# rsadsb/dump1090_rs

Hardware: AMD Instinct MI355X
Metric: IQ Msamples/s demodulated (higher is better)
Workload: dtype i16 IQ -> f32 magnitude (exact) -> u16/i32 integer

## Files before the change

dump1090_rs_amd/csrc/adsb_aux.hip:

```cpp
#include <algorithm>

#include "../../include/adsb_hip.h"
#include "adsb_dev_common.h"
#include "adsb_scan_geometry.h"
#include "adsb_tail_dev.h"
#include "adsb_fix_dev.h"

namespace adsb {

namespace {


__global__ __launch_bounds__(256) void k_to_mag(const uint32_t *__restrict__ iq, uint32_t n,
                                                uint16_t *__restrict__ data)
{
    const uint32_t t = blockIdx.x * 256u + threadIdx.x;
    const uint32_t i0 = 8u * t;
    if (i0 >= (uint32_t)kMagDataLen) return;
    const __amdgpu_buffer_rsrc_t rsrc = __builtin_amdgcn_make_buffer_rsrc((void *)iq, 0, (int)(n * 4u), 0x00020000);
    uint32_t w[8];
#pragma unroll
    for (int i = 0; i < 8; i++) {
        int off = ((int)i0 + i - kLead) * 4;
        asm volatile("" : "+v"(off));
        w[i] = __builtin_amdgcn_raw_buffer_load_b32(rsrc, off, 0, 0);
    }
    uint32_t pk[4];
#pragma unroll
    for (int i = 0; i < 4; i++) pk[i] = mag2(w[2 * i], w[2 * i + 1]);
    if (i0 + 8u <= (uint32_t)kMagDataLen) {
        *(uint4 *)(data + i0) = make_uint4(pk[0], pk[1], pk[2], pk[3]);
    } else {
        for (uint32_t i = 0; i0 + i < (uint32_t)kMagDataLen; i++) data[i0 + i] = (uint16_t)(pk[i >> 1] >> (16 * (i & 1)));
    }
}

__global__ __launch_bounds__(256) void k_to_mag_u8(const uint8_t *__restrict__ iq, uint32_t n, const uint16_t *__restrict__ tab,
                                                   uint16_t *__restrict__ data)
{
    const uint32_t t = blockIdx.x * 256u + threadIdx.x;
    const uint32_t i0 = 8u * t;
    if (i0 >= (uint32_t)kMagDataLen) return;
    const __amdgpu_buffer_rsrc_t rsrc = __builtin_amdgcn_make_buffer_rsrc((void *)iq, 0, (int)(n * 2u), 0x00020000);
    uint32_t w[8];
#pragma unroll
    for (int i = 0; i < 8; i++) w[i] = load_u8_sample(rsrc, (int)i0 + i - kLead, (int)n, tab);
    uint32_t pk[4];
#pragma unroll
    for (int i = 0; i < 4; i++) pk[i] = mag2(w[2 * i], w[2 * i + 1]);
    if (i0 + 8u <= (uint32_t)kMagDataLen) {
        *(uint4 *)(data + i0) = make_uint4(pk[0], pk[1], pk[2], pk[3]);
    } else {
        for (uint32_t i = 0; i0 + i < (uint32_t)kMagDataLen; i++) data[i0 + i] = (uint16_t)(pk[i >> 1] >> (16 * (i & 1)));
    }
}

__global__ __launch_bounds__(256) void k_widen_u8(const uint8_t *__restrict__ src, unsigned long long first, uint32_t count,
                                                  const uint16_t *__restrict__ tab, uint32_t *__restrict__ dst)
{
    const uint32_t i = blockIdx.x * 256u + threadIdx.x;
    if (i >= count) return;
    const uint8_t *b = src + 2ull * (first + i);
    dst[i] = widen_u8_pair(tab, (uint32_t)b[0] | (uint32_t)b[1] << 8);
}

__global__ __launch_bounds__(256) void k_reset(Counters *ctr, uint32_t *bitmap, uint32_t lg)
{
    const uint32_t i = blockIdx.x * blockDim.x + threadIdx.x;
    constexpr uint32_t kCtrDwords = sizeof(Counters) / 4;
    if (i < kCtrDwords) ((uint32_t *)ctr)[i] = 0;
    if (bitmap) bitmap_clear(bitmap, lg, i, gridDim.x * blockDim.x);
}


__global__ __launch_bounds__(256) void k_match(ScanParams p)
{
    if (p.order_cnt) TAIL_PRIO();
    __shared__ uint32_t stab[3 * 256];
    __shared__ uint32_t coarse[kCoarseWords];
    for (int i = threadIdx.x; i < 3 * 256; i += blockDim.x) stab[i] = p.tables[kTabX56 * 256 + i];
    if (threadIdx.x < kCoarseWords) coarse[threadIdx.x] = p.bitmap[bitmap_words(p.bitmap_lg) + threadIdx.x];
    __syncthreads();
    const uint32_t seg_cap = p.seg_cap;
    const bool is_dap = blockIdx.x >= (uint32_t)kApWaveSegs / 2;
    uint32_t n[2];
    const uint64_t *ap[2];
    uint32_t first = 0, stride = 2 * blockDim.x;
    if (is_dap) {
        n[0] = n[1] = min(p.ctr->n_dap, p.dap_cap);
        ap[0] = ap[1] = p.dap;
        first = (blockIdx.x - kApWaveSegs / 2) * 4 * blockDim.x;
        stride = (gridDim.x - kApWaveSegs / 2) * 4 * blockDim.x;
    } else {
        for (int h = 0; h < 2; h++) {
            const uint32_t sg = 2 * blockIdx.x + h;
            n[h] = min(p.ctr->seg_ap[sg], seg_cap);
            ap[h] = p.ap + (uint64_t)sg * seg_cap;
        }
    }
    const uint32_t nmax = max(n[0], n[1]);
    for (uint32_t i0 = first + threadIdx.x; i0 < nmax; i0 += stride) {
        uint64_t e[4];
        uint32_t c[4];
#pragma unroll
        for (int k = 0; k < 4; k++) {
            const int h = is_dap ? 0 : k >> 1;
            const uint32_t i = i0 + (is_dap ? (uint32_t)k : (uint32_t)(k & 1)) * blockDim.x;
            e[k] = i < n[h] ? ap[h][i] : ~0ull;
        }
#pragma unroll
        for (int k = 0; k < 4; k++) {
            const uint32_t code = entry_code(e[k]);
            c[k] = entry_value(e[k]);
            if (code >= 5 && code < 10) c[k] = gf_apply(stab, c[k]);
        }
#pragma unroll
        for (int k = 0; k < 4; k++) {
            if (e[k] == ~0ull || !((coarse[(c[k] & 4095u) >> 5] >> (c[k] & 31)) & 1u)) continue;
            const uint32_t at = bitmap_index(c[k], p.bitmap_lg);
            if ((p.bitmap[at >> 5] >> (at & 31)) & 1u) {
                const uint32_t idx = atomicAdd(&p.ctr->n_hits, 1u);
                if (p.order_cnt) {
                    const uint32_t ch = (uint32_t)entry_chunk(e[k]), tl = entry_j(e[k]) / (uint32_t)fastgeo::kTile;
                    const uint32_t at = atomicAdd(&p.order_cnt[ch * fastgeo::kTilesPerChunk + tl], 1u);
                    if (at < kTileBucket) {
                        const size_t place = (size_t)ch * kOrderBucket + tl * kTileBucket + at;
                        p.order_tmp[place] = e[k];
                        if (p.hit_fields) p.hit_fields[place * kHitFieldWords + 5] = 0u;
                    } else {
                        atomicOr(&p.ctr->overflow, 1u);
                    }
                } else if (idx < p.hits_cap) {
                    p.hits[idx] = e[k];
                    if (p.hit_fields) p.hit_fields[(size_t)idx * kHitFieldWords + 5] = 0u;
                } else {
                    atomicOr(&p.ctr->overflow, 1u);
                }
            }
        }
    }
}


__global__ __launch_bounds__(1024) void k_order_prefix(ScanParams p)
{
    TAIL_PRIO();
    __shared__ uint32_t part[1024];
    __shared__ uint32_t carry;
    const uint32_t tid = threadIdx.x;
    constexpr uint32_t T = fastgeo::kTilesPerChunk;
    if (p.ctr->overflow) {
        for (uint32_t c = tid; c < p.n_chunks * T; c += 1024) p.order_cnt[c] = 0;
        return;
    }
    if (tid == 0) carry = 0;
    __syncthreads();
    for (uint32_t c0 = 0; c0 <= p.n_chunks; c0 += 1024) {
        const uint32_t c = c0 + tid;
        uint32_t v = 0;
        if (c < p.n_chunks)
#pragma unroll
            for (uint32_t t = 0; t < T; t++) v += min(p.order_cnt[c * T + t], kTileBucket);
        part[tid] = v;
        __syncthreads();
        for (uint32_t off = 1; off < 1024; off <<= 1) {
            const uint32_t add = tid >= off ? part[tid - off] : 0u;
            __syncthreads();
            part[tid] += add;
            __syncthreads();
        }
        if (c <= p.n_chunks) p.order_base[c] = carry + part[tid] - v;
        __syncthreads();
        if (tid == 1023) carry += part[1023];
        __syncthreads();
    }
}



__device__ __forceinline__ uint32_t score_hash_first(const ScoreDev &sd, uint32_t v)
{
    uint32_t h = score_hash_slot(v) & sd.hash_mask;
    for (;;) {
        const unsigned long long cur = __hip_atomic_load(&sd.hash[h], __ATOMIC_RELAXED, __HIP_MEMORY_SCOPE_AGENT);
        if (cur == ~0ull) return 0xFFFFFFFFu;
        if ((uint32_t)(cur >> 32) == v) return (uint32_t)cur;
        h = (h + 1u) & sd.hash_mask;
    }
}

__device__ __forceinline__ bool score_in_filter(const ScoreDev &sd, uint32_t v, uint32_t i)
{
    if (v == 0) return true;
    if ((sd.exact[v >> 5] >> (v & 31)) & 1u) return true;
    if (sd.earlier && ((sd.earlier[v >> 5] >> (v & 31)) & 1u)) return true;
    return score_hash_first(sd, v) < i;
}

__device__ __forceinline__ int score_repair(const ScoreDev &sd, uint32_t i, uint32_t damaged, const uint32_t *tables, uint32_t fix,
                                            uint32_t *repair)
{
    const TrialRecord &r = sd.rec[i];
    const uint32_t df = (uint32_t)r.msg[0] >> 3;
    if (df != 17u && df != 18u) return -2;
    const uint32_t ab = fix_lookup(tables, (uint32_t)(r.power >> 40), fix);
    if (ab == kFixNoRepair) return -2;
    *repair = ab;
    const uint32_t a = ab & 0xFFu, b = ab >> 8;
    const uint32_t addr = damaged ^ fix_addr_mask(a) ^ fix_addr_mask(b);
    if (!score_in_filter(sd, addr, i)) return -1;
    return a == kFixNoBit ? ADSB_SCORE_FIXED_1BIT : ADSB_SCORE_FIXED_2BIT;
}

__device__ __forceinline__ int score_trial(const ScoreDev &sd, uint32_t i, uint32_t *adds, const uint32_t *tables, uint32_t fix,
                                           uint32_t *repair)
{
    const uint32_t w = sd.si[i], v = w & 0xFFFFFFu, kind = w >> 24;
    *adds = 0;
    switch (kind) {
    case kSkApShort: return score_in_filter(sd, v, i) ? 1000 : -1;
    case kSkApLong: return score_in_filter(sd, v, i) ? 1000 : -2;
    case kSkDf11: return score_in_filter(sd, v, i) ? 1000 : -1;
    case kSkDf11Iid0:
        if (score_in_filter(sd, v, i)) return 1600;
        *adds = v;
        return 750;
    case kSkDf17:
        if (score_in_filter(sd, v, i)) return 1800;
        *adds = v;
        return 1400;
    case kSkDf18:
        if (score_in_filter(sd, v, i)) return 1800;
        *adds = v | (1u << 25);
        return 1400;
    case kSkNone: return -3;
    case kSkOther: return fix ? score_repair(sd, i, v, tables, fix, repair) : -2;
    default: return -2;
    }
}


__global__ __launch_bounds__(256) void k_score(ScanParams p)
{
    TAIL_PRIO();
    const ScoreDev &sd = p.score;
    const uint32_t n = sd.state->n;
    const uint32_t per = (n + gridDim.x - 1) / gridDim.x;
    const uint32_t first = blockIdx.x * per, last = min(n, first + per);
    uint32_t emits = 0, addc = 0;
    for (uint32_t i = first + threadIdx.x; i < last; i += blockDim.x) {
        const uint64_t pos = sd.pos[i];
        uint32_t g0 = i;
        while (g0 > 0 && i - g0 < 8 && sd.pos[g0 - 1] == pos) g0--;
        int best = -2, mine = -2;
        uint32_t win = 0xFFFFFFFFu, my_add = 0, my_fix = kFixNoRepair;
        for (uint32_t k = g0; k < n && k < g0 + 16 && sd.pos[k] == pos; k++) {
            uint32_t a, fx = kFixNoRepair;
            const int s = score_trial(sd, k, &a, p.tables, p.fix, &fx);
            if (k == i) {
                mine = s;
                my_add = a;
                my_fix = fx;
            }
            if (s > best) {
                best = s;
                win = k;
            }
        }
        const bool emit = win == i && best >= 0;
        const uint32_t fa = my_fix & 0x7Fu, fb = (my_fix >> 8) & 0x7Fu;
        sd.flag[i] = (emit ? 1u : 0u) | (my_add ? 2u : 0u) | ((uint32_t)(mine + 3) << 8) | (fa >> 6) << 2 | (fa & 63u) << 19 | fb << 25;
        emits += emit;
        addc += my_add != 0;
    }
    __shared__ uint32_t tot[2];
    if (threadIdx.x < 2) tot[threadIdx.x] = 0;
    __syncthreads();
    if (emits) atomicAdd(&tot[0], emits);
    if (addc) atomicAdd(&tot[1], addc);
    __syncthreads();
    if (threadIdx.x < 2) sd.blk[2 * blockIdx.x + threadIdx.x] = tot[threadIdx.x];
}

__global__ __launch_bounds__(256) void k_emit(ScanParams p)
{
    TAIL_PRIO();
    const ScoreDev &sd = p.score;
    const uint32_t n = sd.state->n;
    const uint32_t per = (n + gridDim.x - 1) / gridDim.x;
    const uint32_t first = blockIdx.x * per, last = min(n, first + per);
    static_assert(kScoreBlocks == 256, "the block-offset reduction below takes one earlier block per thread");
    __shared__ uint32_t base[2], scan[2][256];
    __shared__ unsigned long long stage[5 * 256];
    __shared__ uint32_t wtot[2][4];
    {
// ... 93 lines not shown
        if (threadIdx.x == 0) {
            base[0] += scan[0][255];
            base[1] += scan[1][255];
        }
        __syncthreads();
    }
    asm volatile("s_waitcnt vmcnt(0)" ::: "memory");
#pragma unroll
    for (int off = 32; off > 0; off >>= 1) my_sum += __shfl_down(my_sum, off);
    if ((threadIdx.x & 63) == 0 && my_sum) atomicAdd(&sd.state->msg_sum, my_sum);
    asm volatile("s_waitcnt vmcnt(0)" ::: "memory");
    __shared__ bool is_last;
    __syncthreads();
    if (threadIdx.x == 0) is_last = atomicAdd(&sd.state->blocks_done, 1u) == gridDim.x - 1;
    __syncthreads();
    if (!is_last) return;
    __shared__ uint32_t tot[2][4];
    {
        uint32_t nm = threadIdx.x < gridDim.x ? sd.blk[2 * threadIdx.x] : 0u;
        uint32_t na = threadIdx.x < gridDim.x ? sd.blk[2 * threadIdx.x + 1] : 0u;
#pragma unroll
        for (int off = 32; off > 0; off >>= 1) {
            nm += __shfl_down(nm, off);
            na += __shfl_down(na, off);
        }
        if ((threadIdx.x & 63) == 0) {
            tot[0][threadIdx.x >> 6] = nm;
            tot[1][threadIdx.x >> 6] = na;
        }
    }
    __syncthreads();
    if (threadIdx.x == 0) {
        const uint32_t nm = tot[0][0] + tot[0][1] + tot[0][2] + tot[0][3];
        const uint32_t na = tot[1][0] + tot[1][1] + tot[1][2] + tot[1][3];
        const unsigned long long ms = atomicAdd(&sd.state->msg_sum, 0ull);
        uint32_t *sm = (uint32_t *)sd.summary;
        const uint32_t vals[8] = {nm, na, (uint32_t)ms, (uint32_t)(ms >> 32), sd.state->scored, 0u, 0u, sd.seq};
#pragma unroll
        for (int k = 0; k < 8; k++) host_store32(sm + k, vals[k]);
        sd.state->n = 0;
        sd.state->scored = 0;
        sd.state->blocks_done = 0;
        sd.state->msg_sum = 0;
    }
}


template <bool FROM_MAG, bool BUCKETS, bool U8 = false>
__global__ __launch_bounds__(256) void k_records(ScanParams p, TrialRecord *rec)
{
    if (p.order_cnt) TAIL_PRIO();
    extern __shared__ uint64_t sorted[];
    records_block<FROM_MAG, BUCKETS, false, U8>(p, rec, blockIdx.x, gridDim.x, sorted, true);
}

__global__ __launch_bounds__(kCarrySamples) void k_update_carry(const uint32_t *__restrict__ prev,
                                                               const uint32_t *__restrict__ src, long long n,
                                                               uint32_t *__restrict__ next)
{
    const long long i = threadIdx.x, idx = n - kCarrySamples + i;
    next[i] = idx >= 0 ? src[idx] : prev[i + n];
}

__global__ __launch_bounds__(kCarrySamples) void k_update_carry_u8(const uint32_t *__restrict__ prev,
                                                                  const uint8_t *__restrict__ src, long long n,
                                                                  const uint16_t *__restrict__ tab, uint32_t *__restrict__ next)
{
    const long long i = threadIdx.x, idx = n - kCarrySamples + i;
    next[i] = idx >= 0 ? widen_u8_pair(tab, (uint32_t)src[2 * idx] | (uint32_t)src[2 * idx + 1] << 8) : prev[i + n];
}

__global__ __launch_bounds__(64) void k_shard_summary(ScanParams p)
{
    if (threadIdx.x != 0) return;
    uint32_t *sm = (uint32_t *)p.summary;
    const uint32_t vals[9] = {p.ctr->n_hits, p.ctr->overflow, p.ctr->fresh_sum, p.ctr->n_fresh, 0u, 0u, 0u, p.seq, 0u};
    host_store32(sm + 9, summary_check(vals));
    host_store32(sm + 8, 0u);
#pragma unroll
    for (int k = 0; k < 8; k++) host_store32(sm + k, vals[k]);
}

__global__ __launch_bounds__(256) void k_set_addresses(const uint32_t *__restrict__ addrs, uint32_t n,
                                                       uint32_t *bitmap, uint32_t lg)
{
    const uint32_t i = blockIdx.x * blockDim.x + threadIdx.x;
    if (i < n) bitmap_set(bitmap, lg, addrs[i] & 0xFFFFFFu);
}

__global__ __launch_bounds__(256) void k_mag_digest(uint32_t first_bits, uint32_t count,
                                                    unsigned long long *out)
{
    unsigned long long sum = 0, h = 0;
    const uint32_t half = (count + 1) / 2;
    for (uint32_t i = blockIdx.x * blockDim.x + threadIdx.x; i < half; i += gridDim.x * blockDim.x) {
        const uint32_t b0 = first_bits + i, b1 = first_bits + i + half;
        const f32x2 x = {__uint_as_float(b0), __uint_as_float(i + half < count ? b1 : 0u)};
        const uint32_t pk = mag_tail2(x);
        const uint32_t u0 = pk & 0xFFFFu, u1 = pk >> 16;
        sum += u0;
        h ^= ((unsigned long long)u0 + 1ull) * (2ull * b0 + 1ull);
        if (i + half < count) {
            sum += u1;
            h ^= ((unsigned long long)u1 + 1ull) * (2ull * b1 + 1ull);
        }
    }
    atomicAdd(&out[0], sum);
    atomicXor(&out[1], h);
}

__global__ __launch_bounds__(256) void k_fix_lookup(const uint32_t *__restrict__ tables, const uint32_t *__restrict__ residuals,
                                                    uint32_t n, uint32_t mode, uint32_t *__restrict__ out)
{
    const uint32_t i = blockIdx.x * blockDim.x + threadIdx.x;
    if (i < n) out[i] = fix_lookup(tables, residuals[i], mode);
}

inline int hip_ok(hipError_t e) { return e == hipSuccess ? 0 : (int)e; }
inline void hip_clear() { (void)hipGetLastError(); }

}

int launch_to_mag(const void *d_iq, uint32_t n, uint16_t *d_data, void *stream, const uint16_t *u8_table)
{
    hip_clear();
    const int blocks = ((kMagDataLen + 7) / 8 + 255) / 256;
    if (u8_table) {
        hipLaunchKernelGGL(k_to_mag_u8, dim3(blocks), dim3(256), 0, (hipStream_t)stream, (const uint8_t *)d_iq, n, u8_table, d_data);
        return hip_ok(hipGetLastError());
    }
    hipLaunchKernelGGL(k_to_mag, dim3(blocks), dim3(256), 0, (hipStream_t)stream,
                       (const uint32_t *)d_iq, n, d_data);
    return hip_ok(hipGetLastError());
}

int launch_widen_u8(const void *d_src, uint64_t first, uint32_t count, const uint16_t *u8_table, uint32_t *dst, void *stream)
{
    hip_clear();
    if (count == 0) return 0;
    hipLaunchKernelGGL(k_widen_u8, dim3((count + 255) / 256), dim3(256), 0, (hipStream_t)stream, (const uint8_t *)d_src,
                       (unsigned long long)first, count, u8_table, dst);
    return hip_ok(hipGetLastError());
}

int launch_reset(Counters *ctr, uint32_t *bitmap, uint32_t bitmap_lg, void *stream)
{
    hip_clear();
    const uint32_t ctr_blocks = (uint32_t)((sizeof(Counters) / 4 + 255) / 256);
    const uint32_t blocks = bitmap ? std::max(ctr_blocks, std::min(512u, bitmap_alloc_words(bitmap_lg) / 4 / 256 + 1u)) : ctr_blocks;
    hipLaunchKernelGGL(k_reset, dim3(blocks), dim3(256), 0, (hipStream_t)stream, ctr, bitmap, bitmap_lg);
    return hip_ok(hipGetLastError());
}

int launch_match(const ScanParams &p, void *stream)
{
    hip_clear();
    const uint32_t blocks = kApWaveSegs / 2 + 64;
    hipLaunchKernelGGL(k_match, dim3(blocks), dim3(256), 0, (hipStream_t)stream, p);
    return hip_ok(hipGetLastError());
}

int launch_records(const ScanParams &p, SrcFormat fmt, TrialRecord *d_rec, void *stream)
{
    hip_clear();
    uint32_t blocks = p.n_chunks + 8u;
    if (blocks > 1024) blocks = 1024;
    if (fmt == SrcFormat::kCu8) {
        if (!p.u8_table) return (int)hipErrorInvalidValue;
        if (p.order_cnt)
            hipLaunchKernelGGL((k_records<false, true, true>), dim3(blocks), dim3(256), kOrderBucket * (sizeof(uint64_t) + sizeof(uint16_t)),
                               (hipStream_t)stream, p, d_rec);
        else
            hipLaunchKernelGGL((k_records<false, false, true>), dim3(blocks), dim3(256), 0, (hipStream_t)stream, p, d_rec);
    } else if (fmt == SrcFormat::kMag)
        hipLaunchKernelGGL((k_records<true, false>), dim3(blocks), dim3(256), 0, (hipStream_t)stream, p, d_rec);
    else if (p.order_cnt)
        hipLaunchKernelGGL((k_records<false, true>), dim3(blocks), dim3(256), kOrderBucket * (sizeof(uint64_t) + sizeof(uint16_t)),
                           (hipStream_t)stream, p, d_rec);
    else
        hipLaunchKernelGGL((k_records<false, false>), dim3(blocks), dim3(256), 0, (hipStream_t)stream, p, d_rec);
    return hip_ok(hipGetLastError());
}

int launch_order_hits(const ScanParams &p, void *stream)
{
    hip_clear();
    if (!p.order_cnt || !p.order_base || !p.order_tmp) return 0;
    hipLaunchKernelGGL(k_order_prefix, dim3(1), dim3(1024), 0, (hipStream_t)stream, p);
    return hip_ok(hipGetLastError());
}

int launch_score(const ScanParams &p, void *stream)
{
    hip_clear();
    if (!p.score.si) return 0;
    hipLaunchKernelGGL(k_score, dim3(kScoreBlocks), dim3(256), 0, (hipStream_t)stream, p);
    hipLaunchKernelGGL(k_emit, dim3(kScoreBlocks), dim3(256), 0, (hipStream_t)stream, p);
    return hip_ok(hipGetLastError());
}

int launch_set_addresses(const uint32_t *d_addrs, uint32_t n, uint32_t *bitmap, uint32_t bitmap_lg, void *stream)
{
    hip_clear();
    if (n == 0) return 0;
    hipLaunchKernelGGL(k_set_addresses, dim3((n + 255) / 256), dim3(256), 0, (hipStream_t)stream, d_addrs, n,
                       bitmap, bitmap_lg);
    return hip_ok(hipGetLastError());
}

int launch_shard_summary(const ScanParams &p, void *stream)
{
    hip_clear();
    hipLaunchKernelGGL(k_shard_summary, dim3(1), dim3(64), 0, (hipStream_t)stream, p);
    return hip_ok(hipGetLastError());
}

int launch_update_carry(const uint32_t *prev, const void *d_src, uint64_t n_samples, uint32_t *next, void *stream,
                        const uint16_t *u8_table)
{
    hip_clear();
    if (u8_table) {
        hipLaunchKernelGGL(k_update_carry_u8, dim3(1), dim3(kCarrySamples), 0, (hipStream_t)stream, prev,
                           (const uint8_t *)d_src, (long long)n_samples, u8_table, next);
        return hip_ok(hipGetLastError());
    }
    hipLaunchKernelGGL(k_update_carry, dim3(1), dim3(kCarrySamples), 0, (hipStream_t)stream, prev,
                       (const uint32_t *)d_src, (long long)n_samples, next);
    return hip_ok(hipGetLastError());
}

int launch_fix_lookup(const uint32_t *tables, const uint32_t *d_residuals, uint32_t n, uint32_t mode, uint32_t *d_out, void *stream)
{
    hip_clear();
    if (n == 0) return 0;
    hipLaunchKernelGGL(k_fix_lookup, dim3((n + 255) / 256), dim3(256), 0, (hipStream_t)stream, tables, d_residuals, n, mode, d_out);
    return hip_ok(hipGetLastError());
}

int launch_mag_digest(uint32_t first_bits, uint32_t count, unsigned long long *d_out, void *stream)
{
    hip_clear();
    hipLaunchKernelGGL(k_mag_digest, dim3(1024), dim3(256), 0, (hipStream_t)stream, first_bits, count,
                       d_out);
    return hip_ok(hipGetLastError());
}

}
```

dump1090_rs_amd/csrc/adsb_context.cpp:

```cpp
#include "adsb_ctx.h"

using namespace adsb::host;

extern "C" {

struct DeviceStreams {
    int device = -1;
    int least = 0, greatest = 0;
    hipStream_t high[2] = {};
    hipStream_t small[kScanStreams] = {};
    hipStream_t low[4] = {};
    int n_low = 0;
    unsigned next_low = 0;
    std::vector<hipStream_t> free_own;
};
std::mutex g_streams_mu;
std::vector<DeviceStreams *> g_device_streams;

hipError_t dedicated_stream(int device, hipStream_t *out)
{
    hipDeviceProp_t prop;
    hipError_t e = hipGetDeviceProperties(&prop, device);
    if (e != hipSuccess) return e;
    std::vector<uint32_t> mask((size_t)(prop.multiProcessorCount + 31) / 32, 0xFFFFFFFFu);
// ... 484 lines not shown
try {
    if (!c) return ADSB_ERR_INVALID;
    if (c->submitted != c->delivered || c->shard_active) return ADSB_ERR_BUSY;
    if (enabled && c->n_receivers) return ADSB_ERR_INVALID;
    ADSB_ON_DEVICE(c);
    c->carry_over = enabled != 0;
    for (int si = 0; si < c->n_slots; si++)
        HIP_TRY(c, hipMemsetAsync(c->slot[si].d_carry, 0, kCarrySamples * sizeof(uint32_t), c->stream));
    HIP_TRY(c, hipMemsetAsync(c->d_carry_next, 0, kCarrySamples * sizeof(uint32_t), c->stream));
    HIP_TRY(c, hipStreamSynchronize(c->stream));
    return ADSB_OK;
} ADSB_ABI_CATCH

int adsb_set_error_correction(adsb_ctx *c, int mode)
try {
    if (!c || (mode != ADSB_FIX_NONE && mode != ADSB_FIX_1BIT && mode != ADSB_FIX_2BIT)) return ADSB_ERR_INVALID;
    if (c->submitted != c->delivered || c->shard_active) return ADSB_ERR_BUSY;
    c->crc.set_fix(mode);
    return ADSB_OK;
} ADSB_ABI_CATCH

int adsb_get_error_correction(const adsb_ctx *c) { return c ? c->crc.fix : ADSB_ERR_INVALID; }

int adsb_set_signal_stats(adsb_ctx *c, int enabled)
try {
    if (!c) return ADSB_ERR_INVALID;
    if (c->submitted != c->delivered || c->shard_active) return ADSB_ERR_BUSY;
    if (enabled) {
        ADSB_ON_DEVICE(c);
        if (int rc = ensure_signal_stats(c)) return rc;
    }
    c->signal_stats = enabled != 0;
    return ADSB_OK;
} ADSB_ABI_CATCH

int adsb_get_signal_stats(const adsb_ctx *c) { return c ? (c->signal_stats ? 1 : 0) : ADSB_ERR_INVALID; }
uint64_t adsb_selftest_signal_launches(const adsb_ctx *c) { return c ? c->sig_launches : 0; }

int adsb_fetch_signal_stats(adsb_ctx *c, adsb_signal_stats *out, size_t cap, size_t *n_out)
try {
    if (!c || (!out && cap)) return ADSB_ERR_INVALID;
    const size_t n = std::min(cap, c->sig_out.size());
    if (n) std::memcpy(out, c->sig_out.data(), n * sizeof(adsb_signal_stats));
    if (n_out) *n_out = c->sig_out.size();
    return c->sig_out.size() > cap ? ADSB_ERR_CAPACITY : ADSB_OK;
} ADSB_ABI_CATCH

int adsb_set_u8_table(adsb_ctx *c, const int16_t *table256)
try {
    if (!c) return ADSB_ERR_INVALID;
    if (c->submitted != c->delivered || c->shard_active) return ADSB_ERR_BUSY;
    ADSB_ON_DEVICE(c);
    int16_t t[256];
    if (table256) std::memcpy(t, table256, sizeof t);
    else soapy_u8_table(t);
    HIP_TRY(c, hipMemcpy(c->d_u8_table, t, sizeof t, hipMemcpyHostToDevice));
    return ADSB_OK;
} ADSB_ABI_CATCH

int adsb_selftest_u8_table(adsb_ctx *c, int16_t *out256)
try {
    if (!out256) return ADSB_ERR_INVALID;
    if (!c) {
        soapy_u8_table(out256);
        return ADSB_OK;
    }
    if (c->submitted != c->delivered || c->shard_active) return ADSB_ERR_BUSY;
    ADSB_ON_DEVICE(c);
    HIP_TRY(c, hipMemcpy(out256, c->d_u8_table, 256 * sizeof(int16_t), hipMemcpyDeviceToHost));
    return ADSB_OK;
} ADSB_ABI_CATCH

int adsb_icao_flush(adsb_ctx *c)
{
    if (!c) return ADSB_ERR_INVALID;
    c->flush_pending = true;
    return ADSB_OK;
}

int adsb_set_receivers(adsb_ctx *c, uint32_t n_receivers)
try {
    if (!c || n_receivers > ADSB_MAX_RECEIVERS || (n_receivers && c->carry_over)) return ADSB_ERR_INVALID;
    if (c->submitted != c->delivered || c->shard_active) return ADSB_ERR_BUSY;
    if (n_receivers == c->n_receivers) return ADSB_OK;
    std::vector<IcaoFilter> filters(n_receivers > 1 ? n_receivers - 1 : 0);
    std::vector<IcaoFilter *> filter_of(n_receivers);
    for (uint32_t r = 0; r < n_receivers; r++) filter_of[r] = r ? &filters[r - 1] : &c->filter;
    for (int si = 0; si < c->n_slots; si++) {
        c->slot[si].rx_map.reserve(n_receivers ? c->max_chunks : 0);
        c->slot[si].rx_map.clear();
        c->slot[si].rx_flush.clear();
    }
    c->rx_flush_next.clear();
    c->rx_filters.swap(filters);
    c->rx_filter_of.swap(filter_of);
    c->n_receivers = n_receivers;
    c->filter.flush();
    c->flush_pending = true;
    c->score_epoch++;
    c->exact_valid = false;
    return ADSB_OK;
} ADSB_ABI_CATCH

int adsb_get_receivers(const adsb_ctx *c) { return c ? (int)c->n_receivers : ADSB_ERR_INVALID; }

int adsb_icao_flush_receiver(adsb_ctx *c, uint32_t receiver)
try {
    if (!c || receiver >= c->n_receivers) return ADSB_ERR_INVALID;
    if (c->submitted == c->collected) c->rx_filter_of[receiver]->flush();
    else c->rx_flush_next.push_back(receiver);
    return ADSB_OK;
} ADSB_ABI_CATCH

int adsb_receiver_filter_table(const adsb_ctx *c, uint32_t receiver, uint32_t *out4096)
try {
    if (!c || !out4096 || receiver >= c->n_receivers) return ADSB_ERR_INVALID;
    if (c->submitted != c->collected) return ADSB_ERR_BUSY;
    c->rx_filter_of[receiver]->store(out4096);
    bool flushed = c->flush_pending;
    for (uint32_t r : c->rx_flush_next) flushed = flushed || r == receiver;
    if (flushed) std::memset(out4096, 0, IcaoFilter::kSize * sizeof(uint32_t));
    return ADSB_OK;
} ADSB_ABI_CATCH

int adsb_selftest_rx_tune(adsb_ctx *c, uint32_t parallel_min)
{
    if (!c) return ADSB_ERR_INVALID;
    if (c->submitted != c->delivered) return ADSB_ERR_BUSY;
    c->rx_parallel_min = parallel_min ? parallel_min : kRxParallelReplayMin;
    return ADSB_OK;
}

int adsb_selftest_rx_counters(const adsb_ctx *c, uint64_t *out4)
{
    if (!c || !out4) return ADSB_ERR_INVALID;
    out4[0] = c->rx_passes, out4[1] = c->rx_pooled, out4[2] = c->rx_reseeds, out4[3] = 0;
    return ADSB_OK;
}

uint64_t adsb_host_sorts(const adsb_ctx *c) { return c ? c->host_sorts : 0; }
uint64_t adsb_host_replays(const adsb_ctx *c) { return c ? c->host_replays : 0; }
uint64_t adsb_host_rematches(const adsb_ctx *c) { return c ? c->rematches : 0; }
int adsb_max_in_flight(const adsb_ctx *c) { return c ? c->n_slots : 0; }

int adsb_get_stats(const adsb_ctx *c, adsb_stats *out)
{
    if (!c || !out) return ADSB_ERR_INVALID;
    *out = c->stats;
    return ADSB_OK;
}

const char *adsb_last_error(const adsb_ctx *c) { return c ? c->last_error.c_str() : ""; }

const char *adsb_version(void) { return "adsb_hip 0.22 gfx950 scan=v9-tile-buckets tail=v7-folded-supersets multi=v3-bounded-waits streams=v2-own-queues stats=v1"; }

}
```

dump1090_rs_amd/csrc/adsb_device.h:

```cpp
#pragma once
#include <hip/hip_runtime.h>
#include <stdint.h>

#include <cstdlib>

#include "adsb_record.h"
#include "adsb_tables.h"

#if defined(ADSB_KERNEL_ACCT) && !defined(ADSB_TUNING)
#define ADSB_TUNING 1
#endif
#ifdef ADSB_TUNING
#define ADSB_STOP_AT(p, n) ((p).debug_stop == (n))
#else
#define ADSB_STOP_AT(p, n) false
#endif

namespace adsb {

inline const char *tuning_env(const char *name)
{
#ifdef ADSB_TUNING
    return std::getenv(name);
#else
// ... 29 lines not shown

struct Counters {
    uint32_t n_hits;
    uint32_t overflow;
    uint32_t scan_blocks_done;
    uint32_t n_dap;
    uint32_t n_cand_simple;
    uint32_t blocks_done;
    uint32_t rec_sum[2];
    uint32_t learned_new;
    uint32_t n_rec;
    uint32_t new_addr[kNewAddrCap];
    uint32_t unordered;
    uint32_t t_start[2];
    uint32_t bitmap_ready;
    uint32_t n_fresh;
    uint32_t fresh_sum;
    uint32_t tile_done[kFusedMaxTiles];
    uint32_t seg_ap[kApWaveSegs];
    uint32_t seg_cand[kApSegments];
};

struct Summary {
    uint32_t n_hits, overflow;
    uint32_t rec_sum_lo;
    uint32_t n_dap;
    uint32_t n_ap_total;
    uint32_t n_cand_total;
    uint32_t rec_sum_hi;
    uint32_t seq;
    uint32_t ticks;
    uint32_t check;
};

__host__ __device__ inline uint32_t summary_check(const uint32_t w[9])
{
    uint32_t x = 0xA5D5B17Cu;
    for (int k = 0; k < 9; k++) x ^= (w[k] << (k + 1)) | (w[k] >> (31 - k));
    return x;
}

constexpr int kTabF = 0, kTabX56 = 3, kTabCount = 6;
constexpr int kTabR16Off = kTabCount * 256, kTabFieldOff = kTabR16Off + 16, kTabBitsOff = kTabFieldOff + 300,
              kTabFixOff = kTabBitsOff + 168,
              kTabFix2Off = (kTabFixOff + kFixSlots + 1 + 3) & ~3,
              kTabWords = kTabFix2Off + kFix2Words;

struct ScoreState {
    uint32_t n;
    uint32_t blocks_done;
    uint32_t scored;
    uint32_t reserved;
    unsigned long long msg_sum;
};
struct ScoreSummary {
    uint32_t n_msgs, n_adds;
    uint32_t msg_sum_lo, msg_sum_hi;
    uint32_t scored;
    uint32_t pad[2];
    uint32_t seq;
};
struct ScoreDev {
    uint32_t cap;
    uint32_t *si;
    TrialRecord *rec;
    unsigned long long *pos;
    uint32_t *flag;
    unsigned long long *hash;
    uint32_t hash_mask;
    uint32_t *slot;
    uint32_t *blk;
    uint32_t *exact;
    const uint32_t *earlier;
    uint32_t *exact_retired;
    ScoreState *state;
    void *out_msgs;
    uint32_t *out_adds;
    ScoreSummary *summary;
    uint32_t seq;
};
constexpr int kScoreBlocks = 256;
enum ScoreKind : uint32_t { kSkOther = 0, kSkApShort, kSkApLong, kSkDf11Iid0, kSkDf11, kSkDf17, kSkDf18, kSkNone };

struct ScanParams {
    const void *src;
    uint64_t n_samples;
    uint32_t n_chunks;
    uint32_t *bitmap;
    uint32_t bitmap_lg;
    uint32_t bitmap_fresh;
    uint64_t *hits;
    uint32_t hits_cap;
    uint64_t *ap;
    uint32_t ap_cap;
    uint32_t seg_cap;
    uint64_t *dap;
    uint32_t dap_cap;
    const uint32_t *tables;
    Counters *ctr;
    uint32_t *clean_bitmap;
    Summary *summary;
    uint32_t seq;
    void *ev_start, *ev_stop;
    uint32_t stagger_ticks;
    int debug_stop;
    unsigned long long *timeline;
    uint32_t keep_counters;
    uint32_t *fresh;
    uint32_t fresh_cap;
    uint32_t *fresh_seen;
    const uint32_t *carry;
    uint32_t lead_from_src;
    uint32_t *order_cnt, *order_base;
    uint64_t *order_tmp;
    uint64_t *cand_out;
    uint32_t *cand_count;
    uint32_t cand_cap;
    ScoreDev score;
    uint32_t *hit_fields;
    TrialRecord *fused_rec;
    const unsigned long long *src_ready;
    uint32_t src_host;
    uint32_t order_polls;
    const uint16_t *u8_table;
    uint32_t fix;
};



constexpr uint32_t kBitmapWords = 1u << 19, kCoarseWords = 128;
constexpr uint32_t kBitmapAllocWords = kBitmapWords + kCoarseWords;
constexpr uint32_t kFullBitmapLg = 24, kSmallBitmapLg = 19;
__host__ __device__ inline uint32_t bitmap_words(uint32_t lg) { return 1u << (lg - 5u); }
__host__ __device__ inline uint32_t bitmap_alloc_words(uint32_t lg) { return bitmap_words(lg) + kCoarseWords; }
__host__ __device__ inline uint32_t bitmap_index(uint32_t a, uint32_t lg)
{
    return lg >= kFullBitmapLg ? a : ((a ^ (a >> lg)) & ((1u << lg) - 1u));
}

constexpr uint32_t kOrderBucket = 1024;
constexpr uint32_t kTileBucket = 56;
constexpr int kCarrySamples = 328;

enum class SrcFormat : uint8_t { kMag, kCs16, kCu8 };
inline uint32_t src_bytes_per_sample(SrcFormat f) { return f == SrcFormat::kCu8 ? 2u : 4u; }

int launch_to_mag(const void *d_iq, uint32_t n, uint16_t *d_data, void *stream, const uint16_t *u8_table = nullptr);
int launch_widen_u8(const void *d_src, uint64_t first, uint32_t count, const uint16_t *u8_table, uint32_t *dst, void *stream);
int launch_reset(Counters *ctr, uint32_t *bitmap, uint32_t bitmap_lg, void *stream);
int launch_scan(const ScanParams &p, SrcFormat fmt, void *stream);
int launch_pass_fused(const ScanParams &p, SrcFormat fmt, void *stream);
int scan_resident_blocks();
int launch_scan_simple(const ScanParams &p, SrcFormat fmt, void *stream);
int launch_match(const ScanParams &p, void *stream);
int launch_records(const ScanParams &p, SrcFormat fmt, TrialRecord *d_rec, void *stream);
int launch_order_hits(const ScanParams &p, void *stream);
int launch_shard_summary(const ScanParams &p, void *stream);
int launch_score(const ScanParams &p, void *stream);
int launch_set_addresses(const uint32_t *d_addrs, uint32_t n, uint32_t *bitmap, uint32_t bitmap_lg, void *stream);
int launch_update_carry(const uint32_t *prev, const void *d_src, uint64_t n_samples, uint32_t *next, void *stream,
                        const uint16_t *u8_table = nullptr);
int launch_mag_digest(uint32_t first_bits, uint32_t count, unsigned long long *d_out, void *stream);

constexpr int kSigHistBins = 60;
constexpr int kSigRecordWords = 68;
constexpr int kSigMaxWgPerChunk = 64;
struct SigParams {
    const void *src;
    uint64_t n_samples;
    uint32_t n_chunks;
    uint32_t wg_per_chunk;
    const uint16_t *u8_table;
    uint32_t *partial;
    uint32_t *ticket;
    void *records;
};
uint32_t signal_stats_wg_per_chunk(uint32_t n_chunks);
int launch_signal_stats(const SigParams &p, SrcFormat fmt, void *stream);
int launch_fix_lookup(const uint32_t *tables, const uint32_t *d_residuals, uint32_t n, uint32_t mode, uint32_t *d_out, void *stream);

}
```

dump1090_rs_amd/csrc/adsb_pass.cpp:

```cpp
#include "adsb_ctx.h"

using namespace adsb::host;

namespace adsb {
namespace host {

int ensure_fallback(adsb_ctx *c)
{
    auto &fb = c->fb;
    if (fb.h_rec_dev) return ADSB_OK;
    if (!fb.d_hits) HIP_TRY(c, hipMalloc((void **)&fb.d_hits, (size_t)kWorstPerChunk * sizeof(uint64_t)));
    if (!fb.d_dap) HIP_TRY(c, hipMalloc((void **)&fb.d_dap, (size_t)kWorstPerChunk * sizeof(uint64_t)));
    if (!fb.h_rec)
        HIP_TRY(c, hipHostMalloc((void **)&fb.h_rec, (size_t)kWorstPerChunk * sizeof(TrialRecord), hipHostMallocMapped | hipHostMallocCoherent));
    HIP_TRY(c, hipHostGetDevicePointer((void **)&fb.h_rec_dev, fb.h_rec, 0));
    return ADSB_OK;
}

int fallback_slot(adsb_ctx *c, const Slot &sl, Slot &tmp)
{
    if (int rc = ensure_fallback(c)) return rc;
    tmp = sl;
    tmp.d_hits = c->fb.d_hits;
    tmp.h_rec = c->fb.h_rec;
// ... 142 lines not shown
    p.timeline = c->d_timeline;
    p.carry = c->carry_over && !pl.from_mag ? sl.d_carry : nullptr;
    p.u8_table = fmt == SrcFormat::kCu8 ? c->d_u8_table : nullptr;
    p.lead_from_src = opt.lead_from_src ? 1u : 0u;
    p.order_cnt = pl.ordered ? sl.d_order_cnt : nullptr;
    p.order_base = pl.ordered ? sl.d_order_base : nullptr;
    p.order_tmp = pl.ordered ? sl.d_order_tmp : nullptr;
    p.hit_fields = pl.fused || (pl.ordered && !knob_no_hit_fields()) ? sl.d_hit_fields : nullptr;
    sl.device_scored = pl.scored;
    if (pl.scored) {
        uint32_t *exact_retired = nullptr;
        if (c->flush_pending) {
            exact_retired = c->exact_bm[c->cur_exact];
            c->cur_exact ^= 1;
        }
        wire_score(sl, p, c->exact_bm[c->cur_exact], exact_retired);
        sl.score_epoch = c->score_epoch;
    }
    p.fused_rec = pl.fused ? sl.h_rec_dev : nullptr;
    p.order_polls = c->order_polls;
    p.src_ready = pl.fused && !pl.from_mag ? c->next_src_ready : nullptr;
    c->next_src_ready = nullptr;
    p.src_host = pl.fused && !pl.from_mag && c->next_src_host && !knob_no_trickle() ? 1u : 0u;
    c->next_src_host = false;
    sl.src = d_src;
    sl.fmt = fmt;
    sl.n_samples = n_samples;
    sl.n_chunks = n_chunks;
    sl.flush_before = c->flush_pending;
    c->flush_pending = false;
    sl.profiled = pl.prof;
    sl.fused = pl.fused;
    sl.unsynced_from = 0;
    stamp_seq(c, sl, p, sl.device_scored);
    sl.redo = opt.redo;
    if (!sl.redo) sl.scan_seq = ++c->scan_counter;
    const hipEvent_t *ev = sl.redo ? c->redo_ev : c->scan_ev[sl.scan_seq % kScanEvRing];
    sl.ev[0] = ev[0], sl.ev[1] = ev[1];
    const bool stamps = knob_ext_events() && pl.prof == 1 && pl.fast && !pl.fused;
    p.ev_start = stamps ? sl.ev[0] : nullptr;
    p.ev_stop = stamps ? sl.ev[1] : nullptr;
}

int order_behind_input(adsb_ctx *c, hipEvent_t input_done, int si, hipStream_t ss)
{
    if (input_done != input_ready_now()) {
        HT(c, HT_IN_READY);
        hipEvent_t ready = input_done;
        const bool nothing_to_wait_for = !ready && c->stream == c->own_stream && !c->own_stream_dirty;
        if (!ready && !nothing_to_wait_for) {
            ready = c->input_ready[si];
            HIP_TRY(c, hipEventRecord(ready, c->stream));
            c->own_stream_dirty = false;
        }
        if (ready) HIP_TRY(c, hipStreamWaitEvent(ss, ready, 0));
    }
    return put_behind(c, ss, c->input_on_stream);
}

static int edges_before_scan(adsb_ctx *c, Slot &sl, const ScanParams &p, const PassPlan &pl)
{
    hipStream_t ss = pl.ss;
    if (int rc = order_behind_fused(c, sl, ss)) return rc;
    sl.fused_q = pl.fused ? ss : nullptr;
    bool behind_fresh = false;
    if (c->bitmap_lg != kFullBitmapLg) {
        const long my_slot = &sl - c->slot;
        if (p.bitmap_fresh) {
            c->fresh_q = ss;
            c->fresh_seq = c->epoch_first_seq = sl.scan_seq;
            c->fresh_slot = my_slot >= 0 && my_slot < kSlots ? (int)my_slot : -1;
        } else if (c->fresh_q && c->fresh_q != ss && c->fresh_slot >= 0 && c->fresh_slot != my_slot) {
            const Slot &f = c->slot[c->fresh_slot];
            if (f.busy && f.scan_seq == c->fresh_seq) {
                if (int rc = put_behind(c, ss, c->fresh_q)) return rc;
                behind_fresh = true;
            }
        }
    }
    if (pl.fused) {
        HT(c, HT_EV_SCANNED);
        if (p.clean_bitmap)
            for (Slot &other : c->slot)
                if (&other != &sl && other.busy && other.tail_q != ss)
                    if (int rc = wait_for_tail_of(c, ss, other)) return rc;
        bool other_stream_synced = false;
        if (c->prev_scan_stream && c->prev_scan_stream != ss && !c->prev_fused && c->prev_scanned) {
            HIP_TRY(c, hipStreamWaitEvent(ss, c->prev_scanned, 0));
            other_stream_synced = true;
        }
        for (Slot &other : c->slot)
            if (&other != &sl && other.busy && other.scan_q != ss && other.scan_seq >= c->epoch_first_seq &&
                !(other_stream_synced && other.scan_q == c->prev_scan_stream) && !(behind_fresh && other.scan_seq == c->fresh_seq))
                sl.unsynced_from = sl.unsynced_from ? std::min(sl.unsynced_from, other.scan_seq) : other.scan_seq;
    }
    sl.scan_q = ss;
    return ADSB_OK;
}

static int launch_scan_step(adsb_ctx *c, Slot &sl, ScanParams &p, SrcFormat fmt, const PassOptions &opt, const PassPlan &pl)
{
    hipStream_t ss = pl.ss;
    if (p.bitmap_fresh && !pl.fused) {
        if (int e = launch_reset(sl.d_ctr, p.bitmap, p.bitmap_lg, ss)) return fail(c, (hipError_t)e, "launch_reset");
        p.bitmap_fresh = 0;
    }
    if (pl.classic) HIP_TRY(c, hipEventRecord(sl.ev[0], ss));
    const bool hand_carry_on = p.carry && !opt.redo;
    if (hand_carry_on)
        HIP_TRY(c, hipMemcpyAsync(sl.d_carry, c->d_carry_next, kCarrySamples * sizeof(uint32_t),
                                  hipMemcpyDeviceToDevice, ss));
    {
        HT(c, HT_SCAN_LAUNCH);
        if (int e = pl.fused ? launch_pass_fused(p, fmt, ss)
                             : (opt.force_simple ? launch_scan_simple(p, fmt, ss) : launch_scan(p, fmt, ss)))
            return fail(c, (hipError_t)e, "launch_scan");
    }
    if (pl.classic) HIP_TRY(c, hipEventRecord(sl.ev[1], ss));
    if (hand_carry_on) {
        if (int e = launch_update_carry(sl.d_carry, p.src, p.n_samples, c->d_carry_next, ss, p.u8_table))
            return fail(c, (hipError_t)e, "launch_update_carry");
    }
    return ADSB_OK;
}

static int enqueue_tail(adsb_ctx *c, Slot &sl, const ScanParams &p, SrcFormat fmt, const PassPlan &pl)
{
    hipStream_t ss = pl.ss;
    hipStream_t ts = pl.inline_tail ? ss : c->tail_stream;
    if (p.clean_bitmap && pl.fast) {
        for (Slot &other : c->slot)
            if (&other != &sl && other.busy && other.tail_q != ts)
                if (int rc = wait_for_tail_of(c, ts, other)) return rc;
    }
    {
        HT(c, HT_EV_SCANNED);
        HIP_TRY(c, hipEventRecord(sl.scanned, ss));
        if (!pl.inline_tail) HIP_TRY(c, hipStreamWaitEvent(ts, sl.scanned, 0));
        if (c->prev_scanned && !c->prev_fused && c->prev_scan_stream != ss && (pl.inline_tail || c->prev_inline))
            HIP_TRY(c, hipStreamWaitEvent(ts, c->prev_scanned, 0));
        for (hipStream_t q : c->scan_stream) {
            if (!q || q == ts || (q == ss && !pl.inline_tail)) continue;
            bool any = false;
            for (Slot &other : c->slot) any = any || (&other != &sl && other.busy && other.fused && other.tail_q == q);
            if (!any) continue;
            if (int rc = put_behind(c, ts, q)) return rc;
        }
    }
    c->prev_scanned = sl.scanned;
    c->prev_scan_stream = ss;
    c->prev_inline = pl.inline_tail;
    c->prev_fused = false;
    if (pl.prof > 1) HIP_TRY(c, hipEventRecord(sl.ev[2], ts));
    {
        HT(c, HT_MATCH_LAUNCH);
        if (!knob_skip_match())
            if (int e = launch_match(p, ts)) return fail(c, (hipError_t)e, "launch_match");
        if (int e = launch_order_hits(p, ts)) return fail(c, (hipError_t)e, "launch_order_hits");
    }
    if (pl.prof > 1) HIP_TRY(c, hipEventRecord(sl.ev[3], ts));
    {
        HT(c, HT_RECORDS_LAUNCH);
        if (int e = launch_records(p, fmt, sl.h_rec_dev, ts)) return fail(c, (hipError_t)e, "launch_records");
    }
    sl.tail_q = ts;
    {
        HT(c, HT_EV_DONE);
        HIP_TRY(c, hipEventRecord(sl.recorded, ts));
    }
    return ADSB_OK;
}

static int enqueue_signal_stats(adsb_ctx *c, Slot &sl, const ScanParams &p, SrcFormat fmt, const PassOptions &opt, const PassPlan &pl)
{
    if (opt.redo) return ADSB_OK;
    sl.sig_on = c->signal_stats && pl.fast && sl.h_sig != nullptr;
    if (!sl.sig_on) return ADSB_OK;
    SigParams sp{};
    sp.src = p.src;
    sp.n_samples = p.n_samples;
    sp.n_chunks = p.n_chunks;
    sp.wg_per_chunk = signal_stats_wg_per_chunk(p.n_chunks);
    sp.u8_table = p.u8_table;
    sp.partial = sl.d_sig_part;
    sp.ticket = sl.d_sig_ticket;
    sp.records = sl.h_sig_dev;
    std::memset(sl.h_sig, 0xFF, (size_t)p.n_chunks * sizeof(adsb_signal_stats));
    if (int e = launch_signal_stats(sp, fmt, pl.ss)) return fail(c, (hipError_t)e, "launch_signal_stats");
    c->sig_launches++;
    return ADSB_OK;
}

static int enqueue_score(adsb_ctx *c, Slot &sl, const ScanParams &p, const PassPlan &pl)
{
    hipStream_t ts = sl.tail_q;
    if (sl.device_scored) {
        hipStream_t qs = c->score_stream;
        HIP_TRY(c, hipStreamWaitEvent(qs, sl.recorded, 0));
        if (int e = launch_score(p, qs)) return fail(c, (hipError_t)e, "launch_score");
        ts = qs;
    }
    if (pl.prof > 1) HIP_TRY(c, hipEventRecord(sl.ev[4], ts));
    {
        HT(c, HT_EV_DONE);
        HIP_TRY(c, hipEventRecord(sl.done, ts));
    }
    return ADSB_OK;
}

int enqueue_pass(adsb_ctx *c, Slot &sl, const void *d_src, SrcFormat fmt, uint64_t n_samples, uint32_t n_chunks,
                 const PassOptions &opt)
{
    PassPlan pl;
    if (int rc = plan_pass(c, sl, fmt, n_chunks, opt, pl)) return rc;
    ScanParams p{};
    fill_pass(c, sl, p, d_src, fmt, n_samples, n_chunks, opt, pl);
    if (int rc = order_behind_input(c, opt.input_done, pl.si, pl.ss)) return rc;
    if (int rc = edges_before_scan(c, sl, p, pl)) return rc;
    if (int rc = enqueue_signal_stats(c, sl, p, fmt, opt, pl)) return rc;
    if (int rc = launch_scan_step(c, sl, p, fmt, opt, pl)) return rc;
    if (pl.fused) {
        sl.tail_q = c->prev_scan_stream = pl.ss;
        c->prev_scanned = nullptr;
        c->prev_inline = c->prev_fused = true;
        return ADSB_OK;
    }
    if (int rc = enqueue_tail(c, sl, p, fmt, pl)) return rc;
    return enqueue_score(c, sl, p, pl);
}

std::vector<uint32_t> filter_addresses(const adsb_ctx *c)
{
    std::vector<uint32_t> addrs;
    for (uint32_t a : c->filter.table())
        if (a != 0 && a <= 0xFFFFFFu) addrs.push_back(a);
    if (c->n_receivers > 1) {
        for (const IcaoFilter &f : c->rx_filters)
            for (uint32_t a : f.table())
                if (a != 0 && a <= 0xFFFFFFu) addrs.push_back(a);
        std::sort(addrs.begin(), addrs.end());
        addrs.erase(std::unique(addrs.begin(), addrs.end()), addrs.end());
    }
    return addrs;
}

int ensure_addrs(adsb_ctx *c, size_t n, size_t alloc)
{
    if (n <= c->addrs_cap) return ADSB_OK;
    if (c->d_addrs) (void)hipFree(c->d_addrs);
    c->d_addrs = nullptr;
    c->addrs_cap = 0;
    HIP_TRY(c, hipMalloc((void **)&c->d_addrs, alloc * sizeof(uint32_t)));
    c->addrs_cap = alloc;
    return ADSB_OK;
}

int resync_exact(adsb_ctx *c)
{
    const std::vector<uint32_t> addrs = filter_addresses(c);
    hipStream_t ts = c->score_stream;
    for (uint32_t *bm : c->exact_bm) HIP_TRY(c, hipMemsetAsync(bm, 0, kBitmapAllocWords * sizeof(uint32_t), ts));
    if (!addrs.empty()) {
        if (int rc = ensure_addrs(c, addrs.size(), IcaoFilter::kSize)) return rc;
        HIP_TRY(c, hipMemcpyAsync(c->d_addrs, addrs.data(), addrs.size() * sizeof(uint32_t), hipMemcpyHostToDevice, ts));
        if (int e = launch_set_addresses(c->d_addrs, (uint32_t)addrs.size(), c->exact_bm[c->cur_exact], kFullBitmapLg, ts))
            return fail(c, (hipError_t)e, "launch_set_addresses");
    }
    HIP_TRY(c, hipStreamSynchronize(ts));
    c->exact_valid = true;
    return ADSB_OK;
}

int reseed_bitmap_from_filter(adsb_ctx *c)
{
    const std::vector<uint32_t> addrs = filter_addresses(c);
    if (addrs.empty()) return ADSB_OK;
    if (c->n_receivers) c->rx_reseeds++;
    if (int rc = ensure_addrs(c, addrs.size(), std::max<size_t>(IcaoFilter::kSize, addrs.size()))) return rc;
    HIP_TRY(c, hipMemcpy(c->d_addrs, addrs.data(), addrs.size() * sizeof(uint32_t), hipMemcpyHostToDevice));
    if (int e = launch_set_addresses(c->d_addrs, (uint32_t)addrs.size(), c->d_bitmap[c->cur_bitmap], c->bitmap_lg, c->scan_stream[0]))
        return fail(c, (hipError_t)e, "launch_set_addresses");
    return ADSB_OK;
}

int submit(adsb_ctx *c, const void *d_src, SrcFormat fmt, uint64_t n_samples, bool inline_tail,
           hipEvent_t input_done)
{
    const uint64_t n_chunks = fmt == SrcFormat::kMag ? 1 : (n_samples + kChunkSamples - 1) / kChunkSamples;
    if (n_chunks == 0 || n_chunks > kMaxChunks || n_chunks > c->max_chunks) return ADSB_ERR_INVALID;
    Slot &sl = c->slot[c->submitted % (uint64_t)c->n_slots];
    if (sl.busy || sl.parked || c->shard_active) return ADSB_ERR_BUSY;
#ifdef ADSB_TUNING
    const auto te0 = std::chrono::steady_clock::now();
#endif
    PassOptions opt;
    opt.inline_tail = inline_tail;
    opt.input_done = input_done;
    int rc = enqueue_pass(c, sl, d_src, fmt, n_samples, (uint32_t)n_chunks, opt);
#ifdef ADSB_TUNING
    c->t_enqueue += std::chrono::duration<double>(std::chrono::steady_clock::now() - te0).count();
#endif
    if (rc) return rc;
    if (c->n_receivers) {
        if (c->rx_call_map) {
            sl.rx_map.assign(c->rx_call_map, c->rx_call_map + n_chunks);
            c->rx_call_map += n_chunks;
        } else {
            sl.rx_map.assign((size_t)n_chunks, 0u);
        }
        sl.rx_flush.clear();
        sl.rx_flush.swap(c->rx_flush_next);
    }
    sl.busy = true;
    c->submitted++;
    return ADSB_OK;
}
// ... 323 lines not shown
```

Before: 721,500.

## Add sparse match kernel over filled segment pairs and shrink records grid

Adds a k_match_sparse kernel that launches one block per filled segment pair, limited to the resident scan blocks. Each block returns early when its pairs' counts are zero, prefetches the next pair's entries, and loops only over the entries that are actually present. This replaces the fixed-size k_match grid that covers all wave segments, in the fast unordered full-bitmap path. The records launch also uses a fixed small grid (72 blocks) in that path for cs16 input, cutting launch and idle-block overhead. The trade-off is less parallelism when hit density is high, and extra control logic in the host path.

```diff
diff --git a/dump1090_rs_amd/csrc/adsb_aux.hip b/dump1090_rs_amd/csrc/adsb_aux.hip
--- a/dump1090_rs_amd/csrc/adsb_aux.hip
+++ b/dump1090_rs_amd/csrc/adsb_aux.hip
@@ -141,6 +141,77 @@
     }
 }
 
+#ifndef ADSB_MATCH_PAIRS
+#define ADSB_MATCH_PAIRS 1
+#endif
+template <int K>
+__global__ __launch_bounds__(256) void k_match_sparse(ScanParams p, uint32_t n_pairs)
+{
+    __shared__ uint32_t stab[3 * 256];
+    __shared__ uint32_t coarse[kCoarseWords];
+    const uint32_t seg_cap = p.seg_cap, tid = threadIdx.x;
+    const uint32_t pair0 = blockIdx.x * (uint32_t)K;
+    uint32_t n[K][2], any = 0;
+#pragma unroll
+    for (int q = 0; q < K; q++)
+#pragma unroll
+        for (int h = 0; h < 2; h++) {
+            n[q][h] = pair0 + q < n_pairs ? min(p.ctr->seg_ap[2 * (pair0 + q) + h], seg_cap) : 0u;
+            any |= n[q][h];
+        }
+    if (!any) return;
+    auto fetch = [&](const uint32_t (&cnt)[2], uint32_t pair, uint32_t base, uint64_t (&e)[4]) {
+#pragma unroll
+        for (int k = 0; k < 4; k++) {
+            const uint32_t i = base + tid + (uint32_t)(k & 1) * 256u;
+            e[k] = i < cnt[k >> 1] ? p.ap[(uint64_t)(2 * pair + (k >> 1)) * seg_cap + i] : ~0ull;
+        }
+    };
+    auto look = [&](const uint64_t (&e)[4]) {
+        uint32_t c[4];
+#pragma unroll
+        for (int k = 0; k < 4; k++) {
+            const uint32_t code = entry_code(e[k]);
+            c[k] = entry_value(e[k]);
+            if (code >= 5 && code < 10) c[k] = gf_apply(stab, c[k]);
+        }
+#pragma unroll
+        for (int k = 0; k < 4; k++) {
+            if (e[k] == ~0ull || !((coarse[(c[k] & 4095u) >> 5] >> (c[k] & 31)) & 1u)) continue;
+            const uint32_t at = bitmap_index(c[k], p.bitmap_lg);
+            if ((p.bitmap[at >> 5] >> (at & 31)) & 1u) {
+                const uint32_t idx = atomicAdd(&p.ctr->n_hits, 1u);
+                if (idx < p.hits_cap) {
+                    p.hits[idx] = e[k];
+                    if (p.hit_fields) p.hit_fields[(size_t)idx * kHitFieldWords + 5] = 0u;
+                } else {
+                    atomicOr(&p.ctr->overflow, 1u);
+                }
+            }
+        }
+    };
+    uint64_t e[4];
+    fetch(n[0], pair0, 0u, e);
+    for (uint32_t i = tid; i < 3 * 256; i += 256) stab[i] = p.tables[kTabX56 * 256 + i];
+    if (tid < kCoarseWords) coarse[tid] = p.bitmap[bitmap_words(p.bitmap_lg) + tid];
+    __syncthreads();
+#pragma unroll
+    for (int q = 0; q < K; q++) {
+        uint64_t nx[4];
+        if (q + 1 < K) fetch(n[q + 1 < K ? q + 1 : q], pair0 + q + 1, 0u, nx);
+        look(e);
+        const uint32_t nmax = max(n[q][0], n[q][1]);
+        for (uint32_t base = 512u; base < nmax; base += 512u) {
+            uint64_t f[4];
+            fetch(n[q], pair0 + q, base, f);
+            look(f);
+        }
+        if (q + 1 < K)
+#pragma unroll
+            for (int k = 0; k < 4; k++) e[k] = nx[k];
+    }
+}
+
 
 __global__ __launch_bounds__(1024) void k_order_prefix(ScanParams p)
 {
@@ -540,19 +611,33 @@
     return hip_ok(hipGetLastError());
 }
 
-int launch_match(const ScanParams &p, void *stream)
-{
-    hip_clear();
+int launch_match(const ScanParams &p, void *stream, bool sparse_fast)
+{
+    hip_clear();
+    if (sparse_fast && ADSB_MATCH_PAIRS && !p.order_cnt) {
+        const uint32_t tiles = p.n_chunks * (uint32_t)fastgeo::kTilesPerChunk;
+        const uint32_t n_pairs = 2u * std::min(tiles, (uint32_t)scan_resident_blocks());
+        constexpr uint32_t K = ADSB_MATCH_PAIRS ? ADSB_MATCH_PAIRS : 1;
+        static_assert(K <= 8, "the fill counts of a block's pairs are held in registers");
+        if (n_pairs == 0) return 0;
+        hipLaunchKernelGGL((k_match_sparse<(int)K>), dim3((n_pairs + K - 1) / K), dim3(256), 0, (hipStream_t)stream, p, n_pairs);
+        return hip_ok(hipGetLastError());
+    }
     const uint32_t blocks = kApWaveSegs / 2 + 64;
     hipLaunchKernelGGL(k_match, dim3(blocks), dim3(256), 0, (hipStream_t)stream, p);
     return hip_ok(hipGetLastError());
 }
 
-int launch_records(const ScanParams &p, SrcFormat fmt, TrialRecord *d_rec, void *stream)
+#ifndef ADSB_REC_SPARSE_BLOCKS
+#define ADSB_REC_SPARSE_BLOCKS 72
+#endif
+
+int launch_records(const ScanParams &p, SrcFormat fmt, TrialRecord *d_rec, void *stream, bool sparse_fast)
 {
     hip_clear();
     uint32_t blocks = p.n_chunks + 8u;
     if (blocks > 1024) blocks = 1024;
+    if (sparse_fast && ADSB_REC_SPARSE_BLOCKS && !p.order_cnt && fmt == SrcFormat::kCs16) blocks = ADSB_REC_SPARSE_BLOCKS;
     if (fmt == SrcFormat::kCu8) {
         if (!p.u8_table) return (int)hipErrorInvalidValue;
         if (p.order_cnt)
diff --git a/dump1090_rs_amd/csrc/adsb_context.cpp b/dump1090_rs_amd/csrc/adsb_context.cpp
--- a/dump1090_rs_amd/csrc/adsb_context.cpp
+++ b/dump1090_rs_amd/csrc/adsb_context.cpp
@@ -660,6 +660,6 @@
 
 const char *adsb_last_error(const adsb_ctx *c) { return c ? c->last_error.c_str() : ""; }
 
-const char *adsb_version(void) { return "adsb_hip 0.22 gfx950 scan=v9-tile-buckets tail=v7-folded-supersets multi=v3-bounded-waits streams=v2-own-queues stats=v1"; }
-
-}
+const char *adsb_version(void) { return "adsb_hip 0.22 gfx950 scan=v9-tile-buckets tail=v8-sparse-lean multi=v3-bounded-waits streams=v2-own-queues stats=v1"; }
+
+}
diff --git a/dump1090_rs_amd/csrc/adsb_device.h b/dump1090_rs_amd/csrc/adsb_device.h
--- a/dump1090_rs_amd/csrc/adsb_device.h
+++ b/dump1090_rs_amd/csrc/adsb_device.h
@@ -205,8 +205,8 @@
 int launch_pass_fused(const ScanParams &p, SrcFormat fmt, void *stream);
 int scan_resident_blocks();
 int launch_scan_simple(const ScanParams &p, SrcFormat fmt, void *stream);
-int launch_match(const ScanParams &p, void *stream);
-int launch_records(const ScanParams &p, SrcFormat fmt, TrialRecord *d_rec, void *stream);
+int launch_match(const ScanParams &p, void *stream, bool sparse_fast = false);
+int launch_records(const ScanParams &p, SrcFormat fmt, TrialRecord *d_rec, void *stream, bool sparse_fast = false);
 int launch_order_hits(const ScanParams &p, void *stream);
 int launch_shard_summary(const ScanParams &p, void *stream);
 int launch_score(const ScanParams &p, void *stream);
diff --git a/dump1090_rs_amd/csrc/adsb_pass.cpp b/dump1090_rs_amd/csrc/adsb_pass.cpp
--- a/dump1090_rs_amd/csrc/adsb_pass.cpp
+++ b/dump1090_rs_amd/csrc/adsb_pass.cpp
@@ -318,16 +318,17 @@
     c->prev_inline = pl.inline_tail;
     c->prev_fused = false;
     if (pl.prof > 1) HIP_TRY(c, hipEventRecord(sl.ev[2], ts));
+    const bool sparse_fast = pl.fast && !pl.ordered && c->bitmap_lg == kFullBitmapLg;
     {
         HT(c, HT_MATCH_LAUNCH);
         if (!knob_skip_match())
-            if (int e = launch_match(p, ts)) return fail(c, (hipError_t)e, "launch_match");
+            if (int e = launch_match(p, ts, sparse_fast)) return fail(c, (hipError_t)e, "launch_match");
         if (int e = launch_order_hits(p, ts)) return fail(c, (hipError_t)e, "launch_order_hits");
     }
     if (pl.prof > 1) HIP_TRY(c, hipEventRecord(sl.ev[3], ts));
     {
         HT(c, HT_RECORDS_LAUNCH);
-        if (int e = launch_records(p, fmt, sl.h_rec_dev, ts)) return fail(c, (hipError_t)e, "launch_records");
+        if (int e = launch_records(p, fmt, sl.h_rec_dev, ts, sparse_fast)) return fail(c, (hipError_t)e, "launch_records");
     }
     sl.tail_q = ts;
     {
```

Result: faster. 776,300 (median of 6 runs) (+7.6%).
